# usnistgov/alignn

Measured on NVIDIA H100. Metric: graphs/sec fwd+bwd, higher is better.
Workload: dtype f32

## Files before the change

alignn_b200/csrc/tc_common.cuh:

```cuda
#pragma once
#include <cuda_bf16.h>
#include <cuda_runtime.h>
#include <stdint.h>

namespace alignn {
namespace tc {

__device__ __forceinline__ uint32_t smem_u32(const void* p) { return (uint32_t)__cvta_generic_to_shared(p); }

__device__ __forceinline__ void mbar_init(uint64_t* bar, uint32_t count) {
  asm volatile("mbarrier.init.shared::cta.b64 [%0], %1;" ::"r"(smem_u32(bar)), "r"(count));
}
__device__ __forceinline__ void mbar_fence_init() { asm volatile("fence.mbarrier_init.release.cluster;" ::: "memory"); }
__device__ __forceinline__ void mbar_arrive(uint64_t* bar) {
  asm volatile("{\n\t.reg .b64 st;\n\tmbarrier.arrive.shared::cta.b64 st, [%0];\n\t}" ::"r"(smem_u32(bar)) : "memory");
}
__device__ __forceinline__ void mbar_arrive_relaxed(uint64_t* bar) {
  asm volatile("{\n\t.reg .b64 st;\n\tmbarrier.arrive.relaxed.cta.shared::cta.b64 st, [%0];\n\t}" ::"r"(smem_u32(bar)) : "memory");
}
__device__ __forceinline__ void mbar_wait(uint64_t* bar, uint32_t parity) {
  const uint32_t addr = smem_u32(bar);
  uint32_t done = 0;
  for (uint32_t spin = 0; !done; ++spin) {
    asm volatile(
        "{\n\t.reg .pred p;\n\t"
        "mbarrier.try_wait.parity.shared::cta.b64 p, [%1], %2;\n\t"
        "selp.u32 %0, 1, 0, p;\n\t}"
        : "=r"(done)
        : "r"(addr), "r"(parity)
        : "memory");
    if (spin > (1u << 26)) __trap();
  }
}

__device__ __forceinline__ void mbar_wait_poll(uint64_t* bar, uint32_t parity) {
  const uint32_t addr = smem_u32(bar);
  uint32_t done = 0;
  for (uint32_t spin = 0; !done; ++spin) {
    asm volatile(
        "{\n\t.reg .pred p;\n\t"
        "mbarrier.test_wait.parity.shared::cta.b64 p, [%1], %2;\n\t"
        "selp.u32 %0, 1, 0, p;\n\t}"
        : "=r"(done)
        : "r"(addr), "r"(parity)
        : "memory");
    if (spin > (1u << 28)) __trap();
  }
}

__device__ __forceinline__ void mbar_arrive_expect_tx(uint64_t* bar, uint32_t bytes) {
  asm volatile("{\n\t.reg .b64 st;\n\tmbarrier.arrive.expect_tx.shared::cta.b64 st, [%0], %1;\n\t}" ::"r"(smem_u32(bar)), "r"(bytes)
               : "memory");
}
__device__ __forceinline__ void bulk_g2s(void* dst_smem, const void* src_gmem, uint32_t bytes, uint64_t* bar) {
  asm volatile("cp.async.bulk.shared::cluster.global.mbarrier::complete_tx::bytes [%0], [%1], %2, [%3];" ::"r"(smem_u32(dst_smem)),
               "l"(src_gmem), "r"(bytes), "r"(smem_u32(bar))
               : "memory");
}

__device__ __forceinline__ void bulk_prefetch_l2(const void* src_gmem, uint32_t bytes) {
  asm volatile("cp.async.bulk.prefetch.L2.global [%0], %1;" ::"l"(src_gmem), "r"(bytes) : "memory");
}

__device__ __forceinline__ void fence_async_smem() { asm volatile("fence.proxy.async.shared::cta;" ::: "memory"); }

__device__ __forceinline__ uint64_t smem_desc(uint32_t saddr, uint32_t lbo_bytes, uint32_t sbo_bytes) {
  uint64_t d = 0;
  d |= (uint64_t)((saddr & 0x3FFFFu) >> 4);
  d |= (uint64_t)((lbo_bytes >> 4) & 0x3FFFu) << 16;
  d |= (uint64_t)((sbo_bytes >> 4) & 0x3FFFu) << 32;
  return d;
}
__device__ __forceinline__ void wgmma_fence() { asm volatile("wgmma.fence.sync.aligned;" ::: "memory"); }
__device__ __forceinline__ void wgmma_commit() { asm volatile("wgmma.commit_group.sync.aligned;" ::: "memory"); }
__device__ __forceinline__ void wgmma_wait_all() { asm volatile("wgmma.wait_group.sync.aligned 0;" ::: "memory"); }
template <int N>
__device__ __forceinline__ void wgmma_wait() { asm volatile("wgmma.wait_group.sync.aligned %0;" ::"n"(N) : "memory"); }

template <int N> struct Wgmma;
template <> struct Wgmma<32> {
  template <int TA, int TB>
  static __device__ __forceinline__ void mma(float (&d)[16], uint64_t a, uint64_t b, uint32_t accumulate) {
    asm volatile(
        "{\n\t.reg .pred p;\n\tsetp.ne.b32 p, %18, 0;\n\t"
        "wgmma.mma_async.sync.aligned.m64n32k16.f32.bf16.bf16 {%0, %1, %2, %3, %4, %5, %6, %7, %8, %9, %10, %11, %12, %13, %14, %15}, %16, %17, p, 1, 1, %19, %20;\n\t}"
        : "+f"(d[0]), "+f"(d[1]), "+f"(d[2]), "+f"(d[3]), "+f"(d[4]), "+f"(d[5]), "+f"(d[6]), "+f"(d[7]), "+f"(d[8]), "+f"(d[9]), "+f"(d[10]), "+f"(d[11]), "+f"(d[12]), "+f"(d[13]), "+f"(d[14]), "+f"(d[15])
        : "l"(a), "l"(b), "r"(accumulate), "n"(TA), "n"(TB));
  }
};

template <> struct Wgmma<64> {
  template <int TA, int TB>
  static __device__ __forceinline__ void mma(float (&d)[32], uint64_t a, uint64_t b, uint32_t accumulate) {
    asm volatile(
        "{\n\t.reg .pred p;\n\tsetp.ne.b32 p, %34, 0;\n\t"
        "wgmma.mma_async.sync.aligned.m64n64k16.f32.bf16.bf16 {%0, %1, %2, %3, %4, %5, %6, %7, %8, %9, %10, %11, %12, %13, %14, %15, %16, %17, %18, %19, %20, %21, %22, %23, %24, %25, %26, %27, %28, %29, %30, %31}, %32, %33, p, 1, 1, %35, %36;\n\t}"
        : "+f"(d[0]), "+f"(d[1]), "+f"(d[2]), "+f"(d[3]), "+f"(d[4]), "+f"(d[5]), "+f"(d[6]), "+f"(d[7]), "+f"(d[8]), "+f"(d[9]), "+f"(d[10]), "+f"(d[11]), "+f"(d[12]), "+f"(d[13]), "+f"(d[14]), "+f"(d[15]), "+f"(d[16]), "+f"(d[17]), "+f"(d[18]), "+f"(d[19]), "+f"(d[20]), "+f"(d[21]), "+f"(d[22]), "+f"(d[23]), "+f"(d[24]), "+f"(d[25]), "+f"(d[26]), "+f"(d[27]), "+f"(d[28]), "+f"(d[29]), "+f"(d[30]), "+f"(d[31])
        : "l"(a), "l"(b), "r"(accumulate), "n"(TA), "n"(TB));
  }
};

template <> struct Wgmma<96> {
  template <int TA, int TB>
  static __device__ __forceinline__ void mma(float (&d)[48], uint64_t a, uint64_t b, uint32_t accumulate) {
    asm volatile(
        "{\n\t.reg .pred p;\n\tsetp.ne.b32 p, %50, 0;\n\t"
        "wgmma.mma_async.sync.aligned.m64n96k16.f32.bf16.bf16 {%0, %1, %2, %3, %4, %5, %6, %7, %8, %9, %10, %11, %12, %13, %14, %15, %16, %17, %18, %19, %20, %21, %22, %23, %24, %25, %26, %27, %28, %29, %30, %31, %32, %33, %34, %35, %36, %37, %38, %39, %40, %41, %42, %43, %44, %45, %46, %47}, %48, %49, p, 1, 1, %51, %52;\n\t}"
        : "+f"(d[0]), "+f"(d[1]), "+f"(d[2]), "+f"(d[3]), "+f"(d[4]), "+f"(d[5]), "+f"(d[6]), "+f"(d[7]), "+f"(d[8]), "+f"(d[9]), "+f"(d[10]), "+f"(d[11]), "+f"(d[12]), "+f"(d[13]), "+f"(d[14]), "+f"(d[15]), "+f"(d[16]), "+f"(d[17]), "+f"(d[18]), "+f"(d[19]), "+f"(d[20]), "+f"(d[21]), "+f"(d[22]), "+f"(d[23]), "+f"(d[24]), "+f"(d[25]), "+f"(d[26]), "+f"(d[27]), "+f"(d[28]), "+f"(d[29]), "+f"(d[30]), "+f"(d[31]), "+f"(d[32]), "+f"(d[33]), "+f"(d[34]), "+f"(d[35]), "+f"(d[36]), "+f"(d[37]), "+f"(d[38]), "+f"(d[39]), "+f"(d[40]), "+f"(d[41]), "+f"(d[42]), "+f"(d[43]), "+f"(d[44]), "+f"(d[45]), "+f"(d[46]), "+f"(d[47])
        : "l"(a), "l"(b), "r"(accumulate), "n"(TA), "n"(TB));
  }
};

template <> struct Wgmma<128> {
  template <int TA, int TB>
  static __device__ __forceinline__ void mma(float (&d)[64], uint64_t a, uint64_t b, uint32_t accumulate) {
    asm volatile(
        "{\n\t.reg .pred p;\n\tsetp.ne.b32 p, %66, 0;\n\t"
        "wgmma.mma_async.sync.aligned.m64n128k16.f32.bf16.bf16 {%0, %1, %2, %3, %4, %5, %6, %7, %8, %9, %10, %11, %12, %13, %14, %15, %16, %17, %18, %19, %20, %21, %22, %23, %24, %25, %26, %27, %28, %29, %30, %31, %32, %33, %34, %35, %36, %37, %38, %39, %40, %41, %42, %43, %44, %45, %46, %47, %48, %49, %50, %51, %52, %53, %54, %55, %56, %57, %58, %59, %60, %61, %62, %63}, %64, %65, p, 1, 1, %67, %68;\n\t}"
        : "+f"(d[0]), "+f"(d[1]), "+f"(d[2]), "+f"(d[3]), "+f"(d[4]), "+f"(d[5]), "+f"(d[6]), "+f"(d[7]), "+f"(d[8]), "+f"(d[9]), "+f"(d[10]), "+f"(d[11]), "+f"(d[12]), "+f"(d[13]), "+f"(d[14]), "+f"(d[15]), "+f"(d[16]), "+f"(d[17]), "+f"(d[18]), "+f"(d[19]), "+f"(d[20]), "+f"(d[21]), "+f"(d[22]), "+f"(d[23]), "+f"(d[24]), "+f"(d[25]), "+f"(d[26]), "+f"(d[27]), "+f"(d[28]), "+f"(d[29]), "+f"(d[30]), "+f"(d[31]), "+f"(d[32]), "+f"(d[33]), "+f"(d[34]), "+f"(d[35]), "+f"(d[36]), "+f"(d[37]), "+f"(d[38]), "+f"(d[39]), "+f"(d[40]), "+f"(d[41]), "+f"(d[42]), "+f"(d[43]), "+f"(d[44]), "+f"(d[45]), "+f"(d[46]), "+f"(d[47]), "+f"(d[48]), "+f"(d[49]), "+f"(d[50]), "+f"(d[51]), "+f"(d[52]), "+f"(d[53]), "+f"(d[54]), "+f"(d[55]), "+f"(d[56]), "+f"(d[57]), "+f"(d[58]), "+f"(d[59]), "+f"(d[60]), "+f"(d[61]), "+f"(d[62]), "+f"(d[63])
        : "l"(a), "l"(b), "r"(accumulate), "n"(TA), "n"(TB));
  }
};

__device__ __forceinline__ void split4(const float4 v, uint2& hi, uint2& lo) {
  const __nv_bfloat162 h01 = __floats2bfloat162_rn(v.x, v.y), h23 = __floats2bfloat162_rn(v.z, v.w);
  const float2 f01 = __bfloat1622float2(h01), f23 = __bfloat1622float2(h23);
  const __nv_bfloat162 l01 = __floats2bfloat162_rn(v.x - f01.x, v.y - f01.y), l23 = __floats2bfloat162_rn(v.z - f23.x, v.w - f23.y);
  hi.x = *reinterpret_cast<const uint32_t*>(&h01); hi.y = *reinterpret_cast<const uint32_t*>(&h23);
  lo.x = *reinterpret_cast<const uint32_t*>(&l01); lo.y = *reinterpret_cast<const uint32_t*>(&l23);
}

}
}
```

alignn_b200/csrc/wgrad_tc.cu:

```cuda
#include <cooperative_groups.h>

#include "common.cuh"
#include "tc_common.cuh"
#include "api_common.h"
#include "alignn_b200.h"

namespace alignn {
namespace wgrad {

constexpr int BK = 32;
constexpr int STAGES = 4;
constexpr int LOAD_WARPS = 8;
constexpr int MMA_WARPS = 8;
constexpr int THREADS = 32 * (MMA_WARPS + LOAD_WARPS);
constexpr uint32_t SBO = 128;
constexpr int kNumSMsWgrad = kNumSMs;
constexpr int PROMOTE_CHUNKS = 8;

__host__ __device__ constexpr int tiles_of(int DA, int DB) { return (DA > 128 ? DA / 128 : 1) * (DB > 128 ? DB / 128 : 1); }

template <int DA, int DB>
struct Cfg {
  static constexpr int TA = DA < 128 ? DA : 128;
  static constexpr int TN = DB <= 128 ? DB : 128;
  static constexpr int NT = DB / TN;
  static constexpr int TILES = tiles_of(DA, DB);
  static constexpr int A_PLANE = 128 * BK * 2;
  static constexpr int B_PLANE = TN * BK * 2;
  static constexpr uint32_t LBO_A = (128 / 8) * 128;
  static constexpr uint32_t LBO_B = (TN / 8) * 128;
  static constexpr int STAGE = 2 * A_PLANE + 2 * B_PLANE;
  static constexpr int PIPE = STAGES * STAGE;
  static constexpr int ACC = MMA_WARPS * 32 * (TN / 2) * 4;
  static constexpr int SMEM = PIPE + ACC + 128;
  static_assert(TILES * TA * TN == DA * DB, "output blocks cover the output");
};

template <int DA, int DB>
struct Pipe {
  using F = Cfg<DA, DB>;
  uint8_t* smem;
  uint64_t* full;
  uint64_t* empty;

  __device__ __forceinline__ void load(const float* __restrict__ Ag, int64_t lda, const float* __restrict__ Bg, int64_t ldb,
                                       int64_t r_begin, int64_t r_end, int nk, int g0, int warp, int lane) {
    const int e_l = (lane >> 1) & 7, oq = (lane >> 4) * 2 + (lane & 1);
    constexpr int JA = (F::TA / 16 + LOAD_WARPS - 1) / LOAD_WARPS, JB = (F::TN / 16 + LOAD_WARPS - 1) / LOAD_WARPS;
    constexpr int NT = 4 * (JA + JB);
    auto load_chunk = [&](float4 (&v)[NT], int kc) {
      const int64_t r0 = r_begin + (int64_t)kc * BK + e_l;
#pragma unroll
      for (int eg = 0; eg < 4; ++eg) {
        const int64_t r = r0 + eg * 8;
        const bool rv = r < r_end;
#pragma unroll
        for (int j = 0; j < JA; ++j) {
          const int og = warp + LOAD_WARPS * j;
          v[eg * (JA + JB) + j] = (rv && og < F::TA / 16) ? __ldcs(reinterpret_cast<const float4*>(Ag + r * lda + (og * 4 + oq) * 4))
                                                          : make_float4(0.f, 0.f, 0.f, 0.f);
        }
#pragma unroll
        for (int j = 0; j < JB; ++j) {
          const int og = warp + LOAD_WARPS * j;
          v[eg * (JA + JB) + JA + j] = (rv && og < F::TN / 16) ? __ldcs(reinterpret_cast<const float4*>(Bg + r * ldb + (og * 4 + oq) * 4))
                                                               : make_float4(0.f, 0.f, 0.f, 0.f);
        }
      }
    };
    auto store_chunk = [&](const float4 (&v)[NT], int gc) {
      const int s = gc % STAGES;
      if (gc >= STAGES) tc::mbar_wait(&empty[s], ((gc / STAGES) - 1) & 1);
      uint8_t* st = smem + s * F::STAGE;
#pragma unroll
      for (int eg = 0; eg < 4; ++eg) {
        const int edge = eg * 8 + e_l;
#pragma unroll
        for (int j = 0; j < JA + JB; ++j) {
          const bool isA = j < JA;
          const int og = warp + LOAD_WARPS * (isA ? j : j - JA);
          if (og < (isA ? F::TA : F::TN) / 16) {
            const int o4 = og * 4 + oq;
            uint2 hi, lo;
            tc::split4(v[eg * (JA + JB) + j], hi, lo);
            const int lbo = isA ? (int)F::LBO_A : (int)F::LBO_B;
            const int plane = isA ? F::A_PLANE : F::B_PLANE;
            uint8_t* base = st + (isA ? 0 : 2 * F::A_PLANE);
            const int off = (o4 >> 1) * (int)SBO + (edge >> 3) * lbo + (edge & 7) * 16 + (o4 & 1) * 8;
            *reinterpret_cast<uint2*>(base + off) = hi;
            *reinterpret_cast<uint2*>(base + plane + off) = lo;
          }
        }
      }
      tc::fence_async_smem();
      __syncwarp();
      if (lane == 0) tc::mbar_arrive(&full[s]);
    };
    float4 b0[NT], b1[NT];
    if (nk > 0) load_chunk(b0, 0);
    for (int kc = 0; kc < nk; kc += 2) {
      if (kc + 1 < nk) load_chunk(b1, kc + 1);
      store_chunk(b0, g0 + kc);
      if (kc + 1 < nk) {
        if (kc + 2 < nk) load_chunk(b0, kc + 2);
        store_chunk(b1, g0 + kc + 1);
      }
    }
  }

  __device__ __forceinline__ void mma(float (&acc)[F::TN / 2], int nk, int g0, int wg, int lane) {
    const uint32_t base0 = tc::smem_u32(smem);
    float* run = reinterpret_cast<float*>(smem + F::PIPE) + wg * 128 + (threadIdx.x & 127);
#pragma unroll
    for (int i = 0; i < F::TN / 2; ++i) { run[i * MMA_WARPS * 32] = 0.f; acc[i] = 0.f; }
    for (int kc = 0; kc < nk; ++kc) {
      const int g = g0 + kc, s = g % STAGES;
      tc::mbar_wait(&full[s], (g / STAGES) & 1);
      const uint32_t base = base0 + s * F::STAGE;
      tc::wgmma_fence();
#pragma unroll
      for (int j = 0; j < BK / 16; ++j) {
        const uint64_t b_hi = tc::smem_desc(base + 2 * F::A_PLANE + j * 2 * F::LBO_B, F::LBO_B, SBO);
        const uint64_t b_lo = tc::smem_desc(base + 2 * F::A_PLANE + F::B_PLANE + j * 2 * F::LBO_B, F::LBO_B, SBO);
        const uint32_t ao = j * 2 * F::LBO_A + wg * 8 * SBO;
        const uint64_t a_hi = tc::smem_desc(base + ao, F::LBO_A, SBO);
        const uint64_t a_lo = tc::smem_desc(base + F::A_PLANE + ao, F::LBO_A, SBO);
        tc::Wgmma<F::TN>::template mma<1, 1>(acc, a_lo, b_hi, 1);
        tc::Wgmma<F::TN>::template mma<1, 1>(acc, a_hi, b_lo, 1);
        tc::Wgmma<F::TN>::template mma<1, 1>(acc, a_hi, b_hi, 1);
      }
      tc::wgmma_commit();
      tc::wgmma_wait_all();
      __syncwarp();
      if (lane == 0) tc::mbar_arrive(&empty[s]);
      if ((kc + 1) % PROMOTE_CHUNKS == 0 || kc + 1 == nk) {
#pragma unroll
        for (int i = 0; i < F::TN / 2; ++i) { run[i * MMA_WARPS * 32] += acc[i]; acc[i] = 0.f; }
      }
    }
#pragma unroll
    for (int i = 0; i < F::TN / 2; ++i) acc[i] = run[i * MMA_WARPS * 32];
  }

  __device__ __forceinline__ static void store(const float (&acc)[F::TN / 2], float* out, int mt, int nt, int warp, int lane) {
#pragma unroll
    for (int h = 0; h < 2; ++h) {
      const int r = (warp >> 2) * 64 + (warp & 3) * 16 + (lane >> 2) + 8 * h;
      if (r >= F::TA) continue;
      const int o = mt * F::TA + r;
#pragma unroll
      for (int j = 0; j < F::TN / 8; ++j) {
        const int c = nt * F::TN + 8 * j + 2 * (lane & 3);
        *reinterpret_cast<float2*>(out + ((int64_t)(c >> 5) * DA + o) * 32 + (c & 31)) = make_float2(acc[4 * j + 2 * h], acc[4 * j + 2 * h + 1]);
      }
    }
  }
};

template <int DA, int DB>
__device__ __forceinline__ void pipe_init(uint8_t* smem, uint64_t* full, uint64_t* empty) {
  using F = Cfg<DA, DB>;
  if (threadIdx.x == 0) {
    for (int s = 0; s < STAGES; ++s) { tc::mbar_init(&full[s], LOAD_WARPS); tc::mbar_init(&empty[s], MMA_WARPS); }
    tc::mbar_fence_init();
  }
  if (F::TA < 128) {
    for (int i = threadIdx.x; i < F::PIPE / 16; i += THREADS) reinterpret_cast<uint4*>(smem)[i] = make_uint4(0, 0, 0, 0);
  }
  tc::fence_async_smem();
  __syncthreads();
}

template <int DA, int DB>
__global__ void __launch_bounds__(THREADS, 1)
wgrad_bf16x3_kernel(const float* __restrict__ A, int64_t lda, const float* __restrict__ B, int64_t ldb, int64_t K,
                    int rows_per_cta, float* __restrict__ partials, float* __restrict__ out, int64_t ld_out) {
  using F = Cfg<DA, DB>;
  extern __shared__ __align__(128) uint8_t smem[];
  uint64_t* full = reinterpret_cast<uint64_t*>(smem + F::PIPE + F::ACC);
  Pipe<DA, DB> pipe{smem, full, full + STAGES};
  const int tid = threadIdx.x, warp = tid >> 5, lane = tid & 31;
  const int cta = blockIdx.x, group = blockIdx.y, mt = blockIdx.z / F::NT, nt = blockIdx.z % F::NT;
  const int64_t r_begin = (int64_t)cta * rows_per_cta;
  const int64_t r_end = (r_begin + rows_per_cta < K) ? r_begin + rows_per_cta : K;
  const int nk = r_end > r_begin ? (int)((r_end - r_begin + BK - 1) / BK) : 0;
  pipe_init<DA, DB>(smem, full, full + STAGES);

  if (warp >= MMA_WARPS) {
    pipe.load(A + (int64_t)group * DA + mt * F::TA, lda, B + nt * F::TN, ldb, r_begin, r_end, nk, 0, warp - MMA_WARPS, lane);
  } else {
    float acc[F::TN / 2];
    pipe.mma(acc, nk, 0, warp >> 2, lane);
    Pipe<DA, DB>::store(acc, partials + ((int64_t)group * gridDim.x + cta) * DA * DB, mt, nt, warp, lane);
  }
  if (out) {
    __threadfence();
    cooperative_groups::this_grid().sync();
    const int ctas = gridDim.x;
    const int64_t rank = (int64_t)blockIdx.z * gridDim.x + cta, parts = (int64_t)gridDim.z * gridDim.x;
    constexpr int64_t tile = (int64_t)DA * DB;
    const float* p = partials + (int64_t)group * ctas * tile;
    for (int64_t idx = (rank * THREADS + tid) * 4; idx < tile; idx += parts * THREADS * 4) {
      float4 s = make_float4(0.f, 0.f, 0.f, 0.f);
      int c = 0;
      for (; c + 16 <= ctas; c += 16) {
        float4 v[16];
#pragma unroll
        for (int u = 0; u < 16; ++u) v[u] = __ldcg(reinterpret_cast<const float4*>(p + (int64_t)(c + u) * tile + idx));
#pragma unroll
        for (int u = 0; u < 16; ++u) { s.x += v[u].x; s.y += v[u].y; s.z += v[u].z; s.w += v[u].w; }
      }
      for (; c < ctas; ++c) {
        const float4 v = __ldcg(reinterpret_cast<const float4*>(p + (int64_t)c * tile + idx));
        s.x += v.x; s.y += v.y; s.z += v.z; s.w += v.w;
      }
      const int64_t o = (idx >> 5) % DA, i = (idx >> 5) / DA * 32 + (idx & 31);
      *reinterpret_cast<float4*>(out + ((int64_t)group * DA + o) * ld_out + i) = s;
    }
  }
}

constexpr int kMaxProblems = 64;
constexpr int kMaxSlabs = 320;

struct Problem {
  const float* A; const float* B; float* out;
  int64_t lda, ldb, ld_out, K;
  int slab_first, slab_count;
};
struct Slab { int prob, chunk_begin, chunks; };
struct Batch {
  Problem prob[kMaxProblems];
  Slab slab[kMaxSlabs];
  int cta_first[kNumSMsWgrad + 1];
  int nprob;
};

template <int DA, int DB>
__global__ void __launch_bounds__(THREADS, 1)
wgrad_batch_kernel(const __grid_constant__ Batch bt, float* __restrict__ partials) {
  using F = Cfg<DA, DB>;
  extern __shared__ __align__(128) uint8_t smem[];
  uint64_t* full = reinterpret_cast<uint64_t*>(smem + F::PIPE + F::ACC);
  Pipe<DA, DB> pipe{smem, full, full + STAGES};
  const int tid = threadIdx.x, warp = tid >> 5, lane = tid & 31;
  const int cta = blockIdx.x, mt = blockIdx.y / F::NT, nt = blockIdx.y % F::NT;
  const int s_first = bt.cta_first[cta], s_last = bt.cta_first[cta + 1];
  pipe_init<DA, DB>(smem, full, full + STAGES);

  int g = 0;
  for (int si = s_first; si < s_last; ++si) {
    const Slab sl = bt.slab[si];
    const Problem& pr = bt.prob[sl.prob];
    const int nk = sl.chunks;
    if (warp >= MMA_WARPS) {
      const int64_t r_begin = (int64_t)sl.chunk_begin * BK;
      const int64_t r_end = (r_begin + (int64_t)sl.chunks * BK < pr.K) ? r_begin + (int64_t)sl.chunks * BK : pr.K;
      pipe.load(pr.A + mt * F::TA, pr.lda, pr.B + nt * F::TN, pr.ldb, r_begin, r_end, nk, g, warp - MMA_WARPS, lane);
    } else {
      float acc[F::TN / 2];
      pipe.mma(acc, nk, g, warp >> 2, lane);
      Pipe<DA, DB>::store(acc, partials + (int64_t)si * DA * DB, mt, nt, warp, lane);
    }
    g += nk;
  }
  __threadfence();
  cooperative_groups::this_grid().sync();
  constexpr int64_t tile = (int64_t)DA * DB;
  constexpr int64_t tile4 = tile / 4;
  const int64_t items = (int64_t)bt.nprob * tile4;
  const int64_t rank = (int64_t)blockIdx.y * gridDim.x + cta, parts = (int64_t)gridDim.y * gridDim.x;
  for (int64_t it = rank * THREADS + tid; it < items; it += parts * THREADS) {
    const int pi = (int)(it / tile4);
    const int64_t idx = (it - (int64_t)pi * tile4) * 4;
    const Problem& pr = bt.prob[pi];
    const float* p = partials + (int64_t)pr.slab_first * tile + idx;
    const int n = pr.slab_count;
    float4 s = make_float4(0.f, 0.f, 0.f, 0.f);
    int c = 0;
    for (; c + 8 <= n; c += 8) {
      float4 v[8];
#pragma unroll
      for (int u = 0; u < 8; ++u) v[u] = __ldcg(reinterpret_cast<const float4*>(p + (int64_t)(c + u) * tile));
#pragma unroll
      for (int u = 0; u < 8; ++u) { s.x += v[u].x; s.y += v[u].y; s.z += v[u].z; s.w += v[u].w; }
    }
    for (; c < n; ++c) {
      const float4 v = __ldcg(reinterpret_cast<const float4*>(p + (int64_t)c * tile));
      s.x += v.x; s.y += v.y; s.z += v.z; s.w += v.w;
    }
    const int64_t o = (idx >> 5) % DA, i = (idx >> 5) / DA * 32 + (idx & 31);
    *reinterpret_cast<float4*>(pr.out + o * pr.ld_out + i) = s;
  }
}

constexpr int kSlabCost = 6;
inline int cut_batch(const int64_t* K, int n, int64_t target, int ctas, Batch* bt) {
  int ns = 0, cta = 0;
  int64_t budget = target;
  if (bt) bt->cta_first[0] = 0;
  for (int p = 0; p < n; ++p) {
    int64_t left = (K[p] + BK - 1) / BK, begin = 0;
    const int first = ns;
    while (left > 0) {
      if (budget <= kSlabCost + 2) {
        if (++cta >= ctas) return -2;
        budget = target;
        if (bt) bt->cta_first[cta] = ns;
      }
      int64_t take = budget - kSlabCost;
      if (take > left) take = left;
      if (ns >= kMaxSlabs) return -1;
      if (bt) { bt->slab[ns].prob = p; bt->slab[ns].chunk_begin = (int)begin; bt->slab[ns].chunks = (int)take; }
      ++ns;
      begin += take; left -= take; budget -= take + kSlabCost;
    }
    if (bt) { bt->prob[p].slab_first = first; bt->prob[p].slab_count = ns - first; }
  }
  if (bt) {
    for (int c = cta + 1; c <= kNumSMsWgrad; ++c) bt->cta_first[c] = ns;
    bt->nprob = n;
  }
  return ns;
}
inline int plan_batch(const int64_t* K, int n, int ctas, Batch* bt) {
  if (n < 1 || n > kMaxProblems) return -1;
  int64_t total = 0;
  for (int p = 0; p < n; ++p) total += (K[p] + BK - 1) / BK + kSlabCost;
  int64_t target = (total + ctas - 1) / ctas;
  if (target < 8 * kSlabCost) target = 8 * kSlabCost;
  for (;;) {
    const int ns = cut_batch(K, n, target, ctas, nullptr);
    if (ns == -1) return -1;
    if (ns >= 0) break;
    target += (target + 31) / 32;
  }
  return cut_batch(K, n, target, ctas, bt);
}

__global__ void wgrad_reduce_kernel(const float* __restrict__ partials, int ctas, int64_t tile, float* __restrict__ out,
                                    int64_t ld_out, int DA, int DB) {
  const int64_t idx = ((int64_t)blockIdx.x * blockDim.x + threadIdx.x) * 4;
  const int g = blockIdx.y;
  if (idx >= tile) return;
  const float* p = partials + (int64_t)g * ctas * tile + idx;
  float4 s = make_float4(0.f, 0.f, 0.f, 0.f);
  for (int c = 0; c < ctas; ++c) {
    const float4 v = __ldcs(reinterpret_cast<const float4*>(p + (int64_t)c * tile));
    s.x += v.x; s.y += v.y; s.z += v.z; s.w += v.w;
  }
  const int64_t o = (idx >> 5) % DA, i = (idx >> 5) / DA * 32 + (idx & 31);
  *reinterpret_cast<float4*>(out + ((int64_t)g * DA + o) * ld_out + i) = s;
}

inline int ctas_for(int64_t K, int groups, int tiles) {
  int per_group = kNumSMsWgrad / (groups * tiles);
  if (per_group < 1) per_group = 1;
  const int64_t chunks = (K + BK - 1) / BK;
  const int64_t want = (chunks + 3) / 4;
  if (want < per_group) per_group = (int)(want < 1 ? 1 : want);
  return per_group;
}

template <int DA, int DB>
int launch(const float* A, int64_t lda, const float* B, int64_t ldb, int64_t K, int groups, float* out, int64_t ld_out,
           float* ws, cudaStream_t st) {
  using F = Cfg<DA, DB>;
  static alignn::DeviceOnce configured; int cfg_dev;
  if (configured.needed(&cfg_dev)) {
    cudaError_t e = cudaFuncSetAttribute(wgrad_bf16x3_kernel<DA, DB>, cudaFuncAttributeMaxDynamicSharedMemorySize, F::SMEM);
    if (e != cudaSuccess) return record_cuda_error((int)e);
    configured.done(cfg_dev);
  }
  const int ctas = ctas_for(K, groups, F::TILES);
  int64_t rows = (K + ctas - 1) / ctas;
  rows = (rows + BK - 1) / BK * BK;
  static int coop_ok = -1;
  if (coop_ok < 0) {
    int dev = 0, sms = 0, per_sm = 0, coop = 0;
    cudaGetDevice(&dev);
    cudaDeviceGetAttribute(&sms, cudaDevAttrMultiProcessorCount, dev);
    cudaDeviceGetAttribute(&coop, cudaDevAttrCooperativeLaunch, dev);
    cudaOccupancyMaxActiveBlocksPerMultiprocessor(&per_sm, wgrad_bf16x3_kernel<DA, DB>, THREADS, F::SMEM);
    coop_ok = (coop && (int64_t)sms * per_sm >= kNumSMsWgrad) ? 1 : 0;
  }
  int rows_i = (int)rows;
  if (coop_ok) {
    float* ws_p = ws;
    void* args[] = {(void*)&A, (void*)&lda, (void*)&B, (void*)&ldb, (void*)&K, (void*)&rows_i, (void*)&ws_p, (void*)&out, (void*)&ld_out};
    cudaError_t e = cudaLaunchCooperativeKernel((const void*)wgrad_bf16x3_kernel<DA, DB>, dim3(ctas, groups, F::TILES), dim3(THREADS), args,
                                                (size_t)F::SMEM, st);
    if (e != cudaSuccess) return record_cuda_error((int)e);
    return check_launch();
  }
  wgrad_bf16x3_kernel<DA, DB><<<dim3(ctas, groups, F::TILES), THREADS, F::SMEM, st>>>(A, lda, B, ldb, K, rows_i, ws, nullptr, 0);
  int rc = check_launch();
  if (rc != ALIGNN_OK) return rc;
  const int64_t tile = (int64_t)DA * DB;
  wgrad_reduce_kernel<<<dim3((unsigned)((tile / 4 + 255) / 256), groups), 256, 0, st>>>(ws, ctas, tile, out, ld_out, DA, DB);
  return check_launch();
}

inline bool shape_ok(int DA, int DB) {
  if (DA == DB) return DA == 32 || DA == 64 || DA == 128 || DA == 256;
  return (DA == 256 && (DB == 64 || DB == 96)) || (DA == 64 && (DB == 96 || DB == 32)) || (DA == 32 && (DB == 64 || DB == 96));
}

}
}

constexpr int kBatchNeedsFallback = -1000;

template <int D>
static int launch_batch(const alignn::wgrad::Batch& bt, float* ws, cudaStream_t st) {
  using namespace alignn::wgrad;
  using F = Cfg<D, D>;
  static alignn::DeviceOnce configured; int cfg_dev;
  if (configured.needed(&cfg_dev)) {
    cudaError_t e = cudaFuncSetAttribute(wgrad_batch_kernel<D, D>, cudaFuncAttributeMaxDynamicSharedMemorySize, F::SMEM);
    if (e != cudaSuccess) return alignn::record_cuda_error((int)e);
    configured.done(cfg_dev);
  }
  void* args[] = {(void*)&bt, (void*)&ws};
  cudaError_t e = cudaLaunchCooperativeKernel((const void*)wgrad_batch_kernel<D, D>, dim3(kNumSMsWgrad / F::TILES, F::TILES), dim3(THREADS), args,
                                              (size_t)F::SMEM, st);
  if (e == cudaErrorCooperativeLaunchTooLarge) {
    (void)cudaGetLastError();
    return kBatchNeedsFallback;
  }
  if (e != cudaSuccess) return alignn::record_cuda_error((int)e);
  return alignn::check_launch();
}

extern "C" {

size_t alignn_b200_wgrad_workspace_bytes(int64_t K, int DA, int DB, int groups) {
  if (K < 0 || groups < 1 || !alignn::wgrad::shape_ok(DA, DB)) return 0;
  return (size_t)alignn::wgrad::ctas_for(K, groups, alignn::wgrad::tiles_of(DA, DB)) * groups * DA * DB * sizeof(float);
}

size_t alignn_b200_wgrad_batch_workspace_bytes(const alignn_b200_wgrad_problem* problems, int n, int D) {
  using namespace alignn::wgrad;
  if (!problems || n < 1 || n > kMaxProblems || !shape_ok(D, D)) return 0;
  int64_t K[kMaxProblems];
  for (int p = 0; p < n; ++p) { if (problems[p].K < 0) return 0; K[p] = problems[p].K; }
  const int ns = plan_batch(K, n, kNumSMsWgrad / tiles_of(D, D), nullptr);
  return ns < 0 ? 0 : (size_t)(ns > 0 ? ns : 1) * D * D * sizeof(float);
}

int alignn_b200_wgrad_batch(const alignn_b200_wgrad_problem* problems, int n, int D, void* workspace, size_t workspace_bytes,
                            alignn_stream_t stream) {
  using namespace alignn::wgrad;
  if (!problems || n < 1) return ALIGNN_ERR_BAD_ARG;
  if (!shape_ok(D, D)) return ALIGNN_ERR_UNSUPPORTED_D;
  if (n > kMaxProblems) return ALIGNN_ERR_BAD_ARG;
  int64_t K[kMaxProblems];
  static thread_local Batch bt;
  for (int p = 0; p < n; ++p) {
    const alignn_b200_wgrad_problem& q = problems[p];
    if (q.K < 0 || !q.out || q.ld_out < D || (q.ld_out % 4) || ((uintptr_t)q.out & 15)) return ALIGNN_ERR_BAD_ARG;
    if (q.K > 0 && (!q.A || !q.B || q.lda < D || q.ldb < D || (q.lda % 4) || (q.ldb % 4) || ((uintptr_t)q.A & 15) || ((uintptr_t)q.B & 15)))
      return ALIGNN_ERR_BAD_ARG;
    if (q.K >= ((int64_t)1 << 31) * BK) return ALIGNN_ERR_BAD_ARG;
    K[p] = q.K;
    bt.prob[p].A = q.A; bt.prob[p].B = q.B; bt.prob[p].out = q.out;
    bt.prob[p].lda = q.lda; bt.prob[p].ldb = q.ldb; bt.prob[p].ld_out = q.ld_out; bt.prob[p].K = q.K;
  }
  const int ns = plan_batch(K, n, kNumSMsWgrad / tiles_of(D, D), &bt);
  if (ns < 0) return ALIGNN_ERR_BAD_ARG;
  if (!workspace || workspace_bytes < (size_t)(ns > 0 ? ns : 1) * D * D * sizeof(float)) return ALIGNN_ERR_WORKSPACE;
  static int coop_ok = -1;
  if (coop_ok < 0) {
    int dev = 0, sms = 0, coop = 0;
    cudaGetDevice(&dev);
    cudaDeviceGetAttribute(&sms, cudaDevAttrMultiProcessorCount, dev);
    cudaDeviceGetAttribute(&coop, cudaDevAttrCooperativeLaunch, dev);
    coop_ok = (coop && sms >= kNumSMsWgrad) ? 1 : 0;
  }
  auto one_by_one = [&]() -> int {
    for (int p = 0; p < n; ++p) {
      const alignn_b200_wgrad_problem& q = problems[p];
      if (workspace_bytes < alignn_b200_wgrad_workspace_bytes(q.K, D, D, 1)) return ALIGNN_ERR_WORKSPACE;
      int rc = alignn_b200_wgrad(q.A, q.lda, q.B, q.ldb, q.K, D, D, 1, q.out, q.ld_out, workspace, workspace_bytes, stream);
      if (rc != ALIGNN_OK) return rc;
    }
    return ALIGNN_OK;
  };
  if (!coop_ok) return one_by_one();
  cudaStream_t st = (cudaStream_t)stream;
  float* ws = reinterpret_cast<float*>(workspace);
  int rc = ALIGNN_ERR_UNSUPPORTED_D;
  switch (D) {
    case 256: rc = launch_batch<256>(bt, ws, st); break;
    case 128: rc = launch_batch<128>(bt, ws, st); break;
    case 64: rc = launch_batch<64>(bt, ws, st); break;
    case 32: rc = launch_batch<32>(bt, ws, st); break;
  }
  if (rc == kBatchNeedsFallback) {
    coop_ok = 0;
    return one_by_one();
  }
  return rc;
}

int alignn_b200_wgrad(const float* A, int64_t lda, const float* B, int64_t ldb, int64_t K, int DA, int DB, int groups,
                      float* out, int64_t ld_out, void* workspace, size_t workspace_bytes, alignn_stream_t stream) {
  using namespace alignn::wgrad;
  if (K < 0 || groups < 1 || !out || ld_out < DB || (ld_out % 4)) return ALIGNN_ERR_BAD_ARG;
  if (!shape_ok(DA, DB)) return ALIGNN_ERR_UNSUPPORTED_D;
  if (K > 0 && (!A || !B || lda < (int64_t)groups * DA || ldb < DB || (lda % 4) || (ldb % 4))) return ALIGNN_ERR_BAD_ARG;
  if (K >= ((int64_t)1 << 31) * BK) return ALIGNN_ERR_BAD_ARG;
  if (!workspace || workspace_bytes < alignn_b200_wgrad_workspace_bytes(K, DA, DB, groups)) return ALIGNN_ERR_WORKSPACE;
  cudaStream_t st = (cudaStream_t)stream;
  float* ws = reinterpret_cast<float*>(workspace);
#define WG(a, b) if (DA == a && DB == b) return launch<a, b>(A, lda, B, ldb, K, groups, out, ld_out, ws, st)
  WG(256, 256); WG(128, 128); WG(64, 64); WG(32, 32);
  WG(256, 64); WG(256, 96); WG(64, 96); WG(64, 32); WG(32, 64); WG(32, 96);
#undef WG
  return ALIGNN_ERR_UNSUPPORTED_D;
}

}
```

Measured before the change: 4142.

## Stage wgrad loads through cp.async ring and overlap wgmma with stage release

Loader warps now issue cp.async 16-byte zero-filled copies of raw fp32 rows into a swizzled three-deep staging ring, then split each into bf16 hi/lo planes. This replaces the register double-buffered __ldcs loads and lets global loads run ahead without holding registers. The MMA loop now waits only for the previous wgmma group, so each stage is released one chunk late and tensor-core work overlaps the next chunk. The bf16 stage count drops from four to two to make room for the fp32 ring in shared memory, which may expose loader stalls. An alignment check on A and B is added.

```diff
diff --git a/alignn_b200/csrc/tc_common.cuh b/alignn_b200/csrc/tc_common.cuh
--- a/alignn_b200/csrc/tc_common.cuh
+++ b/alignn_b200/csrc/tc_common.cuh
@@ -57,6 +57,14 @@
                "l"(src_gmem), "r"(bytes), "r"(smem_u32(bar))
                : "memory");
 }
+
+__device__ __forceinline__ void cp_async16_zfill(void* dst_smem, const void* src_gmem, bool valid) {
+  asm volatile("cp.async.cg.shared.global [%0], [%1], 16, %2;" ::"r"(smem_u32(dst_smem)), "l"(src_gmem), "r"(valid ? 16 : 0)
+               : "memory");
+}
+__device__ __forceinline__ void cp_async_commit() { asm volatile("cp.async.commit_group;" ::: "memory"); }
+template <int N>
+__device__ __forceinline__ void cp_async_wait() { asm volatile("cp.async.wait_group %0;" ::"n"(N) : "memory"); }
 
 __device__ __forceinline__ void bulk_prefetch_l2(const void* src_gmem, uint32_t bytes) {
   asm volatile("cp.async.bulk.prefetch.L2.global [%0], %1;" ::"l"(src_gmem), "r"(bytes) : "memory");
diff --git a/alignn_b200/csrc/wgrad_tc.cu b/alignn_b200/csrc/wgrad_tc.cu
--- a/alignn_b200/csrc/wgrad_tc.cu
+++ b/alignn_b200/csrc/wgrad_tc.cu
@@ -9,7 +9,8 @@
 namespace wgrad {
 
 constexpr int BK = 32;
-constexpr int STAGES = 4;
+constexpr int STAGES = 2;
+constexpr int FSTAGES = 3;
 constexpr int LOAD_WARPS = 8;
 constexpr int MMA_WARPS = 8;
 constexpr int THREADS = 32 * (MMA_WARPS + LOAD_WARPS);
@@ -31,9 +32,15 @@
   static constexpr uint32_t LBO_B = (TN / 8) * 128;
   static constexpr int STAGE = 2 * A_PLANE + 2 * B_PLANE;
   static constexpr int PIPE = STAGES * STAGE;
+  static constexpr int NBA = TA / 32, NBB = TN / 32;
+  static constexpr int FSTAGE = LOAD_WARPS * BK * 128;
+  static constexpr int ACC_OFF = PIPE + FSTAGES * FSTAGE;
   static constexpr int ACC = MMA_WARPS * 32 * (TN / 2) * 4;
-  static constexpr int SMEM = PIPE + ACC + 128;
+  static constexpr int BAR_OFF = ACC_OFF + ACC;
+  static constexpr int SMEM = BAR_OFF + 128;
   static_assert(TILES * TA * TN == DA * DB, "output blocks cover the output");
+  static_assert(SMEM <= 232448, "shared memory budget of one sm_90 CTA");
+  static_assert(TA % 32 == 0 && TN % 32 == 0 && NBA + NBB <= LOAD_WARPS, "one loader warp per 32-channel block");
 };
 
 template <int DA, int DB>
@@ -45,47 +52,45 @@
 
   __device__ __forceinline__ void load(const float* __restrict__ Ag, int64_t lda, const float* __restrict__ Bg, int64_t ldb,
                                        int64_t r_begin, int64_t r_end, int nk, int g0, int warp, int lane) {
+    const bool isA = warp < F::NBA, active = warp < F::NBA + F::NBB;
+    const int cb = isA ? warp : warp - F::NBA;
+    const float* __restrict__ src = (isA ? Ag : Bg) + cb * 32 + (lane & 7) * 4;
+    const int64_t ld = isA ? lda : ldb;
+    uint8_t* blk = smem + F::PIPE + warp * BK * 128;
+    auto fetch = [&](int kc) {
+      if (active && kc < nk) {
+        uint8_t* fs = blk + (kc % FSTAGES) * F::FSTAGE;
+#pragma unroll
+        for (int i = 0; i < BK / 4; ++i) {
+          const int row = i * 4 + (lane >> 3);
+          const int64_t r = r_begin + (int64_t)kc * BK + row;
+          const bool rv = r < r_end;
+          tc::cp_async16_zfill(fs + row * 128 + (((lane & 7) + 2 * row) & 7) * 16, src + (rv ? r : r_begin) * ld, rv);
+        }
+      }
+      tc::cp_async_commit();
+    };
     const int e_l = (lane >> 1) & 7, oq = (lane >> 4) * 2 + (lane & 1);
-    constexpr int JA = (F::TA / 16 + LOAD_WARPS - 1) / LOAD_WARPS, JB = (F::TN / 16 + LOAD_WARPS - 1) / LOAD_WARPS;
-    constexpr int NT = 4 * (JA + JB);
-    auto load_chunk = [&](float4 (&v)[NT], int kc) {
-      const int64_t r0 = r_begin + (int64_t)kc * BK + e_l;
-#pragma unroll
-      for (int eg = 0; eg < 4; ++eg) {
-        const int64_t r = r0 + eg * 8;
-        const bool rv = r < r_end;
-#pragma unroll
-        for (int j = 0; j < JA; ++j) {
-          const int og = warp + LOAD_WARPS * j;
-          v[eg * (JA + JB) + j] = (rv && og < F::TA / 16) ? __ldcs(reinterpret_cast<const float4*>(Ag + r * lda + (og * 4 + oq) * 4))
-                                                          : make_float4(0.f, 0.f, 0.f, 0.f);
-        }
-#pragma unroll
-        for (int j = 0; j < JB; ++j) {
-          const int og = warp + LOAD_WARPS * j;
-          v[eg * (JA + JB) + JA + j] = (rv && og < F::TN / 16) ? __ldcs(reinterpret_cast<const float4*>(Bg + r * ldb + (og * 4 + oq) * 4))
-                                                               : make_float4(0.f, 0.f, 0.f, 0.f);
-        }
-      }
-    };
-    auto store_chunk = [&](const float4 (&v)[NT], int gc) {
-      const int s = gc % STAGES;
+    const int lbo = isA ? (int)F::LBO_A : (int)F::LBO_B, plane = isA ? F::A_PLANE : F::B_PLANE;
+#pragma unroll
+    for (int kc = 0; kc < FSTAGES - 1; ++kc) fetch(kc);
+    for (int kc = 0; kc < nk; ++kc) {
+      fetch(kc + FSTAGES - 1);
+      tc::cp_async_wait<FSTAGES - 1>();
+      __syncwarp();
+      const int gc = g0 + kc, s = gc % STAGES;
       if (gc >= STAGES) tc::mbar_wait(&empty[s], ((gc / STAGES) - 1) & 1);
-      uint8_t* st = smem + s * F::STAGE;
-#pragma unroll
-      for (int eg = 0; eg < 4; ++eg) {
-        const int edge = eg * 8 + e_l;
-#pragma unroll
-        for (int j = 0; j < JA + JB; ++j) {
-          const bool isA = j < JA;
-          const int og = warp + LOAD_WARPS * (isA ? j : j - JA);
-          if (og < (isA ? F::TA : F::TN) / 16) {
-            const int o4 = og * 4 + oq;
+      if (active) {
+        const uint8_t* fs = blk + (kc % FSTAGES) * F::FSTAGE;
+        uint8_t* base = smem + s * F::STAGE + (isA ? 0 : 2 * F::A_PLANE);
+#pragma unroll
+        for (int eg = 0; eg < 4; ++eg) {
+          const int edge = eg * 8 + e_l;
+#pragma unroll
+          for (int h = 0; h < 2; ++h) {
+            const int f = h * 4 + oq, o4 = cb * 8 + f;
             uint2 hi, lo;
-            tc::split4(v[eg * (JA + JB) + j], hi, lo);
-            const int lbo = isA ? (int)F::LBO_A : (int)F::LBO_B;
-            const int plane = isA ? F::A_PLANE : F::B_PLANE;
-            uint8_t* base = st + (isA ? 0 : 2 * F::A_PLANE);
+            tc::split4(*reinterpret_cast<const float4*>(fs + edge * 128 + ((f + 2 * edge) & 7) * 16), hi, lo);
             const int off = (o4 >> 1) * (int)SBO + (edge >> 3) * lbo + (edge & 7) * 16 + (o4 & 1) * 8;
             *reinterpret_cast<uint2*>(base + off) = hi;
             *reinterpret_cast<uint2*>(base + plane + off) = lo;
@@ -95,48 +100,44 @@
       tc::fence_async_smem();
       __syncwarp();
       if (lane == 0) tc::mbar_arrive(&full[s]);
-    };
-    float4 b0[NT], b1[NT];
-    if (nk > 0) load_chunk(b0, 0);
-    for (int kc = 0; kc < nk; kc += 2) {
-      if (kc + 1 < nk) load_chunk(b1, kc + 1);
-      store_chunk(b0, g0 + kc);
-      if (kc + 1 < nk) {
-        if (kc + 2 < nk) load_chunk(b0, kc + 2);
-        store_chunk(b1, g0 + kc + 1);
-      }
     }
   }
 
   __device__ __forceinline__ void mma(float (&acc)[F::TN / 2], int nk, int g0, int wg, int lane) {
     const uint32_t base0 = tc::smem_u32(smem);
-    float* run = reinterpret_cast<float*>(smem + F::PIPE) + wg * 128 + (threadIdx.x & 127);
+    float* run = reinterpret_cast<float*>(smem + F::ACC_OFF) + wg * 128 + (threadIdx.x & 127);
 #pragma unroll
     for (int i = 0; i < F::TN / 2; ++i) { run[i * MMA_WARPS * 32] = 0.f; acc[i] = 0.f; }
-    for (int kc = 0; kc < nk; ++kc) {
-      const int g = g0 + kc, s = g % STAGES;
-      tc::mbar_wait(&full[s], (g / STAGES) & 1);
-      const uint32_t base = base0 + s * F::STAGE;
-      tc::wgmma_fence();
-#pragma unroll
-      for (int j = 0; j < BK / 16; ++j) {
-        const uint64_t b_hi = tc::smem_desc(base + 2 * F::A_PLANE + j * 2 * F::LBO_B, F::LBO_B, SBO);
-        const uint64_t b_lo = tc::smem_desc(base + 2 * F::A_PLANE + F::B_PLANE + j * 2 * F::LBO_B, F::LBO_B, SBO);
-        const uint32_t ao = j * 2 * F::LBO_A + wg * 8 * SBO;
-        const uint64_t a_hi = tc::smem_desc(base + ao, F::LBO_A, SBO);
-        const uint64_t a_lo = tc::smem_desc(base + F::A_PLANE + ao, F::LBO_A, SBO);
-        tc::Wgmma<F::TN>::template mma<1, 1>(acc, a_lo, b_hi, 1);
-        tc::Wgmma<F::TN>::template mma<1, 1>(acc, a_hi, b_lo, 1);
-        tc::Wgmma<F::TN>::template mma<1, 1>(acc, a_hi, b_hi, 1);
-      }
-      tc::wgmma_commit();
+    for (int k0 = 0; k0 < nk; k0 += PROMOTE_CHUNKS) {
+      const int k1 = k0 + PROMOTE_CHUNKS < nk ? k0 + PROMOTE_CHUNKS : nk;
+      int prev = -1;
+      for (int kc = k0; kc < k1; ++kc) {
+        const int g = g0 + kc, s = g % STAGES;
+        tc::mbar_wait(&full[s], (g / STAGES) & 1);
+        const uint32_t base = base0 + s * F::STAGE;
+        tc::wgmma_fence();
+#pragma unroll
+        for (int j = 0; j < BK / 16; ++j) {
+          const uint64_t b_hi = tc::smem_desc(base + 2 * F::A_PLANE + j * 2 * F::LBO_B, F::LBO_B, SBO);
+          const uint64_t b_lo = tc::smem_desc(base + 2 * F::A_PLANE + F::B_PLANE + j * 2 * F::LBO_B, F::LBO_B, SBO);
+          const uint32_t ao = j * 2 * F::LBO_A + wg * 8 * SBO;
+          const uint64_t a_hi = tc::smem_desc(base + ao, F::LBO_A, SBO);
+          const uint64_t a_lo = tc::smem_desc(base + F::A_PLANE + ao, F::LBO_A, SBO);
+          tc::Wgmma<F::TN>::template mma<1, 1>(acc, a_lo, b_hi, 1);
+          tc::Wgmma<F::TN>::template mma<1, 1>(acc, a_hi, b_lo, 1);
+          tc::Wgmma<F::TN>::template mma<1, 1>(acc, a_hi, b_hi, 1);
+        }
+        tc::wgmma_commit();
+        tc::wgmma_wait<1>();
+        __syncwarp();
+        if (lane == 0 && prev >= 0) tc::mbar_arrive(&empty[prev]);
+        prev = s;
+      }
       tc::wgmma_wait_all();
       __syncwarp();
-      if (lane == 0) tc::mbar_arrive(&empty[s]);
-      if ((kc + 1) % PROMOTE_CHUNKS == 0 || kc + 1 == nk) {
-#pragma unroll
-        for (int i = 0; i < F::TN / 2; ++i) { run[i * MMA_WARPS * 32] += acc[i]; acc[i] = 0.f; }
-      }
+      if (lane == 0) tc::mbar_arrive(&empty[prev]);
+#pragma unroll
+      for (int i = 0; i < F::TN / 2; ++i) { run[i * MMA_WARPS * 32] += acc[i]; acc[i] = 0.f; }
     }
 #pragma unroll
     for (int i = 0; i < F::TN / 2; ++i) acc[i] = run[i * MMA_WARPS * 32];
@@ -177,7 +178,7 @@
                     int rows_per_cta, float* __restrict__ partials, float* __restrict__ out, int64_t ld_out) {
   using F = Cfg<DA, DB>;
   extern __shared__ __align__(128) uint8_t smem[];
-  uint64_t* full = reinterpret_cast<uint64_t*>(smem + F::PIPE + F::ACC);
+  uint64_t* full = reinterpret_cast<uint64_t*>(smem + F::BAR_OFF);
   Pipe<DA, DB> pipe{smem, full, full + STAGES};
   const int tid = threadIdx.x, warp = tid >> 5, lane = tid & 31;
   const int cta = blockIdx.x, group = blockIdx.y, mt = blockIdx.z / F::NT, nt = blockIdx.z % F::NT;
@@ -241,7 +242,7 @@
 wgrad_batch_kernel(const __grid_constant__ Batch bt, float* __restrict__ partials) {
   using F = Cfg<DA, DB>;
   extern __shared__ __align__(128) uint8_t smem[];
-  uint64_t* full = reinterpret_cast<uint64_t*>(smem + F::PIPE + F::ACC);
+  uint64_t* full = reinterpret_cast<uint64_t*>(smem + F::BAR_OFF);
   Pipe<DA, DB> pipe{smem, full, full + STAGES};
   const int tid = threadIdx.x, warp = tid >> 5, lane = tid & 31;
   const int cta = blockIdx.x, mt = blockIdx.y / F::NT, nt = blockIdx.y % F::NT;
@@ -508,7 +509,9 @@
   using namespace alignn::wgrad;
   if (K < 0 || groups < 1 || !out || ld_out < DB || (ld_out % 4)) return ALIGNN_ERR_BAD_ARG;
   if (!shape_ok(DA, DB)) return ALIGNN_ERR_UNSUPPORTED_D;
-  if (K > 0 && (!A || !B || lda < (int64_t)groups * DA || ldb < DB || (lda % 4) || (ldb % 4))) return ALIGNN_ERR_BAD_ARG;
+  if (K > 0 && (!A || !B || lda < (int64_t)groups * DA || ldb < DB || (lda % 4) || (ldb % 4) || ((uintptr_t)A & 15) ||
+                ((uintptr_t)B & 15)))
+    return ALIGNN_ERR_BAD_ARG;
   if (K >= ((int64_t)1 << 31) * BK) return ALIGNN_ERR_BAD_ARG;
   if (!workspace || workspace_bytes < alignn_b200_wgrad_workspace_bytes(K, DA, DB, groups)) return ALIGNN_ERR_WORKSPACE;
   cudaStream_t st = (cudaStream_t)stream;
```

Result: faster. 4443 (median of 6 runs) (+7.3%).
